# ska-sa/dc_sand

Hardware: AMD Instinct MI355X
Metric: Gcoeff/s (complex weights) 64ant x 1024beam x 32768chan per GPU (higher is better)
Workload: dtype f32

## Files before the change

dc_sand_amd/csrc/bf_capi.hip:

```cpp

#include "../../include/dcs_beamformer.h"
#ifdef DCS_PROBES
#include "../../include/dcs_probes.h"
#endif

#include <hip/hip_runtime.h>

#include <cmath>
#include <cstdio>
#include <cstdlib>
#include <cstring>
#include <new>

#include "../../include/dcs_stream_staging.h"
#include "bf_kernels.h"
#include "bf_ctx_ext.h"
#include "bf_stream_ext.h"

static_assert(sizeof(dcs_delay_vals) == 16, "delay_vals must be 4 x fp32 (BeamformerParameters.h:61-66)");

#define DCS_TRY(expr)                          \
    do {                                       \
        hipError_t _e = (expr);                \
        if (_e != hipSuccess) return (int)_e;  \
    } while (0)

namespace {

constexpr uint32_t kDtSlotFloats = 4096;
constexpr int kDtSlots = 8;

inline hipStream_t as_stream(void *s) { return reinterpret_cast<hipStream_t>(s); }

#define DCS_CHECK_DEVICE(c)                                                \
    do {                                                                   \
        int _cur = -1;                                                     \
        if (hipGetDevice(&_cur) != hipSuccess || _cur != (c)->device) return DCS_ERR_WRONG_DEVICE; \
    } while (0)

bool params_ok(const dcs_bf_params *p)
{
    if (!p) return false;
    if (p->nr_channels < 1 || p->nr_channels > (1 << 24)) return false;
    if (p->nr_stations < 1 || p->nr_beams < 1) return false;
    if ((uint64_t)p->nr_stations * (uint64_t)p->nr_beams > 0x7fffffffull) return false;
    if (!(p->sampling_period > 0.0f) || !std::isfinite(p->sampling_period)) return false;
    if (p->fft_size < 1) return false;
    if (p->nr_samples_per_channel < 1 || p->accumulations_before_new_coeffs < 1) return false;
    if (!(p->adc_sample_rate > 0.0) || !std::isfinite(p->adc_sample_rate)) return false;
    const float D = p->sampling_period * (float)p->nr_channels;
    if (!(D >= 0x1p-40f && D <= 0x1p40f)) return false;
    return true;
}

dcs_bf_consts make_consts(const dcs_bf_params *p)
{
    dcs_bf_consts k;
    volatile float D = p->sampling_period * (float)p->nr_channels;
    volatile float y = 1.0f / D;
    k.fDenominator = D;
    k.fRcpDenominator = y;
    const double scale = (double)(p->nr_channels - 1) * 3.14159274101257324219 / (double)D;
    k.fRotBoundScale = (float)(scale * 1.0001) ;
    if (!(k.fRotBoundScale >= 0.0f)) k.fRotBoundScale = INFINITY;
    k.uDiv3Exact = 0u;
    k.fLowDegLimit = 500.0f;
    k.uHalfMath = 0u;
    k.dHalfChannels = p->nr_channels / 2.0;
    k.dDenominator = (double)D;
    return k;
}

int verify_div3(dcs_bf_consts *k)
{
    uint32_t *d_cnt = nullptr;
    uint32_t h_cnt = 1;
    hipError_t e = hipMalloc((void **)&d_cnt, sizeof(uint32_t));
    if (e != hipSuccess) return (int)e;
    e = hipMemset(d_cnt, 0, sizeof(uint32_t));
    if (e == hipSuccess) e = bf_launch_verify_div3(k->fDenominator, k->fRcpDenominator, d_cnt, nullptr);
    if (e == hipSuccess) e = hipMemcpy(&h_cnt, d_cnt, sizeof(uint32_t), hipMemcpyDeviceToHost);
    (void)hipFree(d_cnt);
    if (e != hipSuccess) return (int)e;
    k->uDiv3Exact = (h_cnt == 0u) ? 1u : 0u;
    return DCS_OK;
}

}

constexpr int kSideStreams = 4;
struct dcs_bf_context {
    bf_ctx_ext_head ext;
    dcs_bf_params p;
    dcs_bf_consts k;
    uint32_t n_pairs;
    int device;
    uint32_t div3_verified;
    bool tuning_now;
    dcs_delay_vals *d_table[2];
    int cur;
    bool table_set;
    float *d_dt;
    float *h_dt;
    hipEvent_t dt_ev[kDtSlots];
    hipStream_t side[kSideStreams];
    hipEvent_t fork_ev, join_ev[kSideStreams];
    bool dt_used[kDtSlots];
    int dt_next;
    uint32_t pairs_pad;
    uint32_t terms_steps;
    float *d_terms;
    uint32_t *d_flags;
    uint32_t flag_epoch;
    float *d_wnorm;
    float *d_wscale;
    float *d_tt_terms;
    uint32_t *d_tt_flags;
    dcs_bf_tuning tune;
    struct tuned_geom {
        bool valid;
        int32_t tpb, cpb, wpc;
    } tuned[3][2];
#ifdef DCS_PROBES
    dcs_probe_knobs probe;
#endif
};
#ifdef DCS_PROBES
#define DCS_PROBE_KNOB(c, f) ((c)->probe.f)
#else
#define DCS_PROBE_KNOB(c, f) 0
#endif

constexpr int kTableRing = 4;
struct dcs_bf_stream {
    bf_stream_ext_head ext;
    dcs_bf_context *ctx;
    hipStream_t stream;
    hipGraph_t graph;
    hipGraphExec_t exec;
    hipGraphNode_t node;
    bf_kernel_launch launch;
    bool has_terms;
    hipGraphNode_t terms_node;
    bf_terms_args terms_args;
    const void *terms_func;
    dim3 terms_grid, terms_block;
    dcs_delay_vals *h_table[kTableRing];
    hipEvent_t table_copied[kTableRing];
    bool table_pending[kTableRing];
    int table_next;
    hipGraph_t ggraph;
    hipGraphExec_t gexec;
    hipGraphNode_t gnode_gather, gnode_terms, gnode_gen;
    bf_gather_launch gather;
    dcs_delay_vals *d_spare;
    hipStream_t stage_stream;
    hipEvent_t staged_ev;
    hipEvent_t released_ev;
    bool released_recorded;
    bool staged;
};

extern "C" {

const char *dcs_error_string(int status)
{
    switch (status) {
    case DCS_OK: return "dcs: success";
    case DCS_ERR_INVALID_ARGUMENT: return "dcs error: invalid argument";
    case DCS_ERR_UNSUPPORTED: return "dcs error: this kernel does not support the requested mode";
    case DCS_ERR_NOT_READY: return "dcs error: not ready (no delay table set)";
    case DCS_ERR_OUT_OF_RANGE: return "dcs error: out of range";
    case DCS_ERR_NO_DEVICE: return "dcs error: no HIP device";
    case DCS_ERR_WRONG_DEVICE: return "dcs error: the context belongs to another device than the current one (dcs_device_set)";
    default: break;
    }
    if (status > 0) return hipGetErrorString((hipError_t)status);
    return "dcs error: unknown status";
}

int dcs_abi_version(void) { return DCS_BF_ABI_VERSION; }

int dcs_bf_default_params(dcs_bf_params *p)
{
    if (!p) return DCS_ERR_INVALID_ARGUMENT;
    p->nr_channels = 64;
    p->nr_stations = 64;
    p->nr_beams = 16;
    p->nr_samples_per_channel = 256;
    p->sampling_period = 1e-7f;
    p->fft_size = 8192;
    p->adc_sample_rate = 1712e6;
    p->accumulations_before_new_coeffs = 256;
    p->reserved = 0;
    return DCS_OK;
}

int dcs_bf_output_bytes(const dcs_bf_params *p, int bitwidth, uint32_t nt, size_t *bytes)
{
    if (!params_ok(p) || !bytes) return DCS_ERR_INVALID_ARGUMENT;
    if (bitwidth != DCS_BF_B16 && bitwidth != DCS_BF_B32) return DCS_ERR_INVALID_ARGUMENT;
    const size_t elem = bitwidth == DCS_BF_B16 ? sizeof(uint16_t) : sizeof(float);
    *bytes = (size_t)nt * (size_t)p->nr_channels * (size_t)p->nr_stations * (size_t)p->nr_beams * 2u * elem;
    return DCS_OK;
}

int dcs_bf_delta_times(const dcs_bf_params *p, uint64_t t0, uint32_t nt, float *dt_out)
{
    if (!params_ok(p) || (!dt_out && nt)) return DCS_ERR_INVALID_ARGUMENT;
    for (uint32_t i = 0; i < nt; i++) {
        const uint64_t t = t0 + i;
        volatile float a = (float)t;
        volatile float b = a * p->sampling_period;
        volatile float c = b * 1e9f;
        volatile float d = c * (float)p->fft_size;
        if (!(d < 9.2e18f)) return DCS_ERR_OUT_OF_RANGE;
        const long step_ns = (long)d;
        volatile float num = (float)step_ns;
        volatile float q = num / 1e9f;
        volatile float dt = 0.0f + q;
        dt_out[i] = dt;
    }
    return DCS_OK;
}

int dcs_bf_ts_diff(const struct timespec *first, const struct timespec *last, float *dt_out)
{
    if (!first || !last || !dt_out) return DCS_ERR_INVALID_ARGUMENT;
    volatile float fl = (float)last->tv_sec, ff = (float)first->tv_sec;
    volatile float secs = fl - ff;
    const long nanosec_difference = last->tv_nsec - first->tv_nsec;
    volatile float num = (float)nanosec_difference;
    volatile float q = num / 1e9f;
    volatile float dt = secs + q;
    *dt_out = dt;
    return DCS_OK;
}

int dcs_bf_simulate_input(const dcs_bf_params *p, dcs_delay_vals *out)
{
    if (!params_ok(p) || !out) return DCS_ERR_INVALID_ARGUMENT;
    const size_t n = (size_t)p->nr_stations * (size_t)p->nr_beams;
    for (size_t i = 0; i < n; i++) {
        volatile float ratio = (float)i / (float)n;
        volatile float ramp = ratio * p->sampling_period;
        out[i].fDelay_s = (float)((double)ramp / 3.0);
        out[i].fDelayRate_sps = (float)2e-6;
        volatile float inv = 1.0f - ratio;
        volatile float ramp2 = inv * p->sampling_period;
        out[i].fPhase_rad = (float)((double)ramp2 / 3.0);
        out[i].fPhaseRate_radps = (float)3e-6;
    }
    return DCS_OK;
}

int dcs_device_count(int *count)
{
    if (!count) return DCS_ERR_INVALID_ARGUMENT;
    *count = 0;
    hipError_t e = hipGetDeviceCount(count);
    if (e == hipErrorNoDevice) { *count = 0; return DCS_OK; }
    return (int)e;
}
int dcs_device_set(int device) { return (int)hipSetDevice(device); }
int dcs_device_synchronize(void) { return (int)hipDeviceSynchronize(); }
int dcs_device_name(int device, char *buf, size_t buflen)
{
    if (!buf || buflen == 0) return DCS_ERR_INVALID_ARGUMENT;
    hipDeviceProp_t prop;
    DCS_TRY(hipGetDeviceProperties(&prop, device));
    std::snprintf(buf, buflen, "%s (%s, %d CUs)", prop.name, prop.gcnArchName, prop.multiProcessorCount);
    return DCS_OK;
}
int dcs_malloc(void **dptr, size_t bytes)
{
    if (!dptr) return DCS_ERR_INVALID_ARGUMENT;
    return (int)hipMalloc(dptr, bytes);
}
int dcs_free(void *dptr) { return (int)hipFree(dptr); }
int dcs_host_alloc(void **hptr, size_t bytes)
{
    if (!hptr) return DCS_ERR_INVALID_ARGUMENT;
    return (int)hipHostMalloc(hptr, bytes, hipHostMallocDefault);
}
int dcs_host_free(void *hptr) { return (int)hipHostFree(hptr); }
int dcs_memcpy_htod(void *dptr, const void *hptr, size_t bytes, void *stream)
{
    return (int)hipMemcpyAsync(dptr, hptr, bytes, hipMemcpyHostToDevice, as_stream(stream));
}
int dcs_memcpy_dtoh(void *hptr, const void *dptr, size_t bytes, void *stream)
{
    return (int)hipMemcpyAsync(hptr, dptr, bytes, hipMemcpyDeviceToHost, as_stream(stream));
}
int dcs_memcpy_dtod(void *dst, const void *src, size_t bytes, void *stream)
{
    return (int)hipMemcpyAsync(dst, src, bytes, hipMemcpyDeviceToDevice, as_stream(stream));
}
int dcs_memcpy2d_dtoh(void *hptr, size_t dst_pitch, const void *dptr, size_t src_pitch, size_t row_bytes,
                      size_t nrows, void *stream)
{
    return (int)hipMemcpy2DAsync(hptr, dst_pitch, dptr, src_pitch, row_bytes, nrows, hipMemcpyDeviceToHost,
                                 as_stream(stream));
}
int dcs_memset(void *dptr, int value, size_t bytes, void *stream)
{
    return (int)hipMemsetAsync(dptr, value, bytes, as_stream(stream));
}
int dcs_stream_create(void **stream)
{
    if (!stream) return DCS_ERR_INVALID_ARGUMENT;
    hipStream_t s;
    DCS_TRY(hipStreamCreateWithFlags(&s, hipStreamNonBlocking));
    *stream = s;
    return DCS_OK;
}
int dcs_stream_destroy(void *stream) { return (int)hipStreamDestroy(as_stream(stream)); }
int dcs_stream_synchronize(void *stream) { return (int)hipStreamSynchronize(as_stream(stream)); }

int dcs_event_create(void **event)
{
    if (!event) return DCS_ERR_INVALID_ARGUMENT;
    hipEvent_t e;
    DCS_TRY(hipEventCreate(&e));
    *event = e;
    return DCS_OK;
}
int dcs_event_destroy(void *event) { return (int)hipEventDestroy(reinterpret_cast<hipEvent_t>(event)); }
int dcs_event_record(void *event, void *stream)
{
    return (int)hipEventRecord(reinterpret_cast<hipEvent_t>(event), as_stream(stream));
}
int dcs_event_synchronize(void *event) { return (int)hipEventSynchronize(reinterpret_cast<hipEvent_t>(event)); }
int dcs_event_elapsed_ms(void *start, void *stop, float *ms)
{
    if (!ms) return DCS_ERR_INVALID_ARGUMENT;
    return (int)hipEventElapsedTime(ms, reinterpret_cast<hipEvent_t>(start), reinterpret_cast<hipEvent_t>(stop));
}

namespace {
int prepare_tiled(dcs_bf_context *c, bool out16, const float *dt_dev, float dt0, uint32_t nt, uint32_t c0, uint32_t nc, void *d_out,
                  bf_kernel_launch *l, const float *dt_host, bool terms_table);
int generate_and_beamform_weighted_impl(dcs_bf_context *c, const float *dt, uint64_t t0, uint32_t nt, const int8_t *d_antenna,
                                        size_t antenna_bytes, const float *d_weights, float *d_beams, size_t beams_bytes,
                                        void *stream);
int beamform_accumulated_weighted_impl(dcs_bf_context *c, const float *dt_coeff, uint64_t t_coeff, uint32_t nt,
                                       const int8_t *d_antenna, size_t antenna_bytes, const float *d_weights, float *d_beams,
                                       size_t beams_bytes, void *stream);
const bf_ctx_ext_ops kWeightsOps = {BF_CTX_EXT_VERSION, generate_and_beamform_weighted_impl, beamform_accumulated_weighted_impl};
}

int dcs_bf_create(const dcs_bf_params *p, dcs_bf_context **out)
{
    if (!out) return DCS_ERR_INVALID_ARGUMENT;
    *out = nullptr;
    if (!params_ok(p)) return DCS_ERR_INVALID_ARGUMENT;
    int ndev = 0;
    if (hipGetDeviceCount(&ndev) != hipSuccess || ndev < 1) return DCS_ERR_NO_DEVICE;
    dcs_bf_context *c = new (std::nothrow) dcs_bf_context();
    if (!c) return (int)hipErrorOutOfMemory;
    std::memset(c, 0, sizeof(*c));
    c->ext.ops = &kWeightsOps;
    c->p = *p;
    c->k = make_consts(p);
    c->n_pairs = (uint32_t)p->nr_stations * (uint32_t)p->nr_beams;
    c->pairs_pad = (c->n_pairs + 255u) & ~255u;
    {
        const uint64_t per_step = (uint64_t)c->pairs_pad * 8u;
        uint64_t steps = (64ull << 20) / per_step;
        if (steps < 1) steps = 1;
        if (steps > kDtSlotFloats) steps = kDtSlotFloats;
        c->terms_steps = (uint32_t)steps;
    }
    c->tune.nontemporal = -1;
    c->tune.xcd_remap = -1;
    c->tune.rows_same_tile = -1;
    int st = DCS_OK;
    do {
        if ((st = (int)hipGetDevice(&c->device)) != 0) break;
        if ((st = (int)bf_warm_module()) != 0) break;
        if ((st = (int)bf_warm_module_mfma()) != 0) break;
        const size_t tb = (size_t)c->n_pairs * sizeof(dcs_delay_vals);
        if ((st = (int)hipMalloc((void **)&c->d_table[0], tb)) != 0) break;
        if ((st = (int)hipMalloc((void **)&c->d_table[1], tb)) != 0) break;
        const size_t db = (size_t)kDtSlots * kDtSlotFloats * sizeof(float);
        if ((st = (int)hipMalloc((void **)&c->d_dt, db)) != 0) break;
        if ((st = (int)hipMalloc((void **)&c->d_tt_terms, (size_t)kTermsInline * c->pairs_pad * 8u)) != 0) break;
        if ((st = (int)hipMalloc((void **)&c->d_tt_flags, (size_t)kTermsInline * (c->pairs_pad / 64u) * 4u)) != 0) break;
        if ((st = (int)hipHostMalloc((void **)&c->h_dt, db, hipHostMallocDefault)) != 0) break;
        for (int i = 0; i < kDtSlots && st == 0; i++) st = (int)hipEventCreateWithFlags(&c->dt_ev[i], hipEventDisableTiming);
        if (st != 0) break;
        for (int i = 0; i < kSideStreams && st == 0; i++) {
            st = (int)hipStreamCreateWithFlags(&c->side[i], hipStreamNonBlocking);
            if (st == 0) st = (int)hipEventCreateWithFlags(&c->join_ev[i], hipEventDisableTiming);
        }
        if (st == 0) st = (int)hipEventCreateWithFlags(&c->fork_ev, hipEventDisableTiming);
        if (st != 0) break;
        c->h_dt[0] = 0.0f;
        if ((st = (int)hipMemcpy(c->d_dt, c->h_dt, sizeof(float), hipMemcpyHostToDevice)) != 0) break;
        if ((st = verify_div3(&c->k)) != 0) break;
        c->div3_verified = c->k.uDiv3Exact;
        for (int w = 0; w < 2; w++) {
            bf_kernel_launch l;
            const uint32_t nt_all = (uint32_t)(c->p.nr_samples_per_channel < (int)kDtInline ? c->p.nr_samples_per_channel : (int)kDtInline);
            float dts[kDtInline] = {0.0f};
            if (prepare_tiled(c, w == 1, nullptr, 0.0f, nt_all > 0 ? nt_all : 1u, 0, (uint32_t)c->p.nr_channels, nullptr, &l, dts, false) == DCS_OK && l.func) {
                hipFuncAttributes attr;
                (void)hipFuncGetAttributes(&attr, l.func);
            }
        }
    } while (0);
    if (st != 0) {
        dcs_bf_destroy(c);
        return st;
    }
    *out = c;
    return DCS_OK;
}

int dcs_bf_destroy(dcs_bf_context *c)
{
    if (!c) return DCS_OK;
    (void)hipFree(c->d_table[0]);
    (void)hipFree(c->d_table[1]);
    (void)hipFree(c->d_dt);
    (void)hipFree(c->d_terms);
    (void)hipFree(c->d_flags);
    (void)hipFree(c->d_wnorm);
    (void)hipFree(c->d_wscale);
    (void)hipFree(c->d_tt_terms);
    (void)hipFree(c->d_tt_flags);
    if (c->h_dt) (void)hipHostFree(c->h_dt);
    for (int i = 0; i < kDtSlots; i++)
        if (c->dt_ev[i]) (void)hipEventDestroy(c->dt_ev[i]);
    for (int i = 0; i < kSideStreams; i++) {
        if (c->join_ev[i]) (void)hipEventDestroy(c->join_ev[i]);
        if (c->side[i]) (void)hipStreamDestroy(c->side[i]);
    }
    if (c->fork_ev) (void)hipEventDestroy(c->fork_ev);
    delete c;
    return DCS_OK;
}

int dcs_bf_upload_delays(dcs_bf_context *c, const dcs_delay_vals *table, void *stream)
{
    if (!c || !table) return DCS_ERR_INVALID_ARGUMENT;
    DCS_CHECK_DEVICE(c);
    const int nxt = c->table_set ? (c->cur ^ 1) : c->cur;
    DCS_TRY(hipMemcpyAsync(c->d_table[nxt], table, (size_t)c->n_pairs * sizeof(dcs_delay_vals),
                           hipMemcpyHostToDevice, as_stream(stream)));
    c->cur = nxt;
    c->table_set = true;
    return DCS_OK;
}

int dcs_bf_set_delays_from_global(dcs_bf_context *c, const void *d_global, uint32_t nb_total,
                                  uint32_t beam_offset, void *stream)
{
    if (!c || !d_global) return DCS_ERR_INVALID_ARGUMENT;
    DCS_CHECK_DEVICE(c);
    if ((uint64_t)beam_offset + (uint64_t)c->p.nr_beams > nb_total) return DCS_ERR_OUT_OF_RANGE;
    if ((reinterpret_cast<uintptr_t>(d_global) & 15u) != 0) return DCS_ERR_INVALID_ARGUMENT;
    const int nxt = c->table_set ? (c->cur ^ 1) : c->cur;
// ... 691 lines not shown
    a.k = c->k;
    a.fp32_chain = (c->tune.math_mode & 8) ? 1u : 0u;
#ifdef DCS_PROBES
    auto knob = [](int32_t v, const char *env) { const char *e = std::getenv(env); return (uint32_t)(v ? v : (e ? std::atoi(e) : 0)); };
    a.max_rounds = knob(c->probe.bacc_rounds, "DCS_BACC_ROUNDS");
    a.probe = knob(c->probe.bacc_probe, "DCS_BACC_PROBE");
    a.unstaged = knob(c->probe.bacc_unstaged, "DCS_BACC_UNSTAGED");
    a.plain_stores = knob(c->probe.bacc_plain, "DCS_BACC_PLAIN");
    a.no_share = knob(c->probe.bacc_no_share, "DCS_BACC_NOSHARE");
    a.wg_per_cu = knob(c->probe.bacc_wg_per_cu, "DCS_BACC_WPC");
    a.order = knob(c->probe.bacc_order, "DCS_BACC_ORDER");
    a.nbt_force = knob(c->probe.bacc_nbt, "DCS_BACC_NBT");
    a.nw_force = knob(c->probe.bacc_waves, "DCS_BACC_WAVES");
#endif
    return (int)(d_weights ? bf_launch_beamform_acc_weighted(a, wa, s) : bf_launch_beamform_acc(a, s));
}

int generate_and_beamform_weighted_impl(dcs_bf_context *c, const float *dt, uint64_t t0, uint32_t nt, const int8_t *d_antenna,
                                        size_t antenna_bytes, const float *d_weights, float *d_beams, size_t beams_bytes,
                                        void *stream)
{
    if (!c || !weights_ok(d_weights)) return DCS_ERR_INVALID_ARGUMENT;
    if (!dt && t0 % 16u) return DCS_ERR_INVALID_ARGUMENT;
    return beamform_impl(c, dt_source{dt, dt ? 0 : t0}, nt, d_antenna, antenna_bytes, d_beams, beams_bytes, stream, d_weights);
}

int beamform_accumulated_weighted_impl(dcs_bf_context *c, const float *dt_coeff, uint64_t t_coeff, uint32_t nt,
                                       const int8_t *d_antenna, size_t antenna_bytes, const float *d_weights, float *d_beams,
                                       size_t beams_bytes, void *stream)
{
    if (!c || !weights_ok(d_weights)) return DCS_ERR_INVALID_ARGUMENT;
    return beamform_acc_impl(c, dt_source{dt_coeff, dt_coeff ? 0 : t_coeff}, nt, d_antenna, antenna_bytes, d_beams, beams_bytes,
                             stream, d_weights);
}
}

int dcs_bf_beamform_accumulated(dcs_bf_context *c, uint64_t t_coeff, uint32_t nt, const int8_t *d_antenna, size_t antenna_bytes,
                                float *d_beams, size_t beams_bytes, void *stream)
{
    return beamform_acc_impl(c, dt_source{nullptr, t_coeff}, nt, d_antenna, antenna_bytes, d_beams, beams_bytes, stream);
}

int dcs_bf_beamform_accumulated_dt(dcs_bf_context *c, float dt_coeff, uint32_t nt, const int8_t *d_antenna, size_t antenna_bytes,
                                   float *d_beams, size_t beams_bytes, void *stream)
{
    return beamform_acc_impl(c, dt_source{&dt_coeff, 0}, nt, d_antenna, antenna_bytes, d_beams, beams_bytes, stream);
}

int dcs_bf_autotune(dcs_bf_context *c, int bitwidth, void *d_out, size_t out_bytes, void *stream,
                    dcs_bf_tuning *chosen)
{
    if (!c || !d_out) return DCS_ERR_INVALID_ARGUMENT;
    DCS_CHECK_DEVICE(c);
    if (bitwidth != DCS_BF_B16 && bitwidth != DCS_BF_B32) return DCS_ERR_INVALID_ARGUMENT;
    if (!c->table_set) return DCS_ERR_NOT_READY;
    const bool out16 = bitwidth == DCS_BF_B16;
    const size_t row = (size_t)c->n_pairs * (out16 ? 4u : 8u);
    uint64_t nc64 = out_bytes / row;
    if (nc64 > (uint64_t)c->p.nr_channels) nc64 = (uint64_t)c->p.nr_channels;
    if (nc64 == 0) return DCS_ERR_INVALID_ARGUMENT;
    const uint32_t nc = (uint32_t)nc64;
    uint64_t nt64 = out_bytes / (row * nc);
    if (nt64 > kDtInline) nt64 = kDtInline;
    const uint32_t nt_tune = nc == (uint32_t)c->p.nr_channels && nt64 > 1 ? (uint32_t)nt64 : 1u;
    hipStream_t s = as_stream(stream);
    {
        const int cap = refuse_if_capturing(s);
        if (cap != DCS_OK) return cap;
    }
    dcs_bf_context::tuned_geom &slot =
        c->tuned[tuned_slot(c, out16)][want_terms_table(c, out16, shape_default_geometry(c, out16, nc, nt_tune), nc, nt_tune) ? 1 : 0];

    auto report = [&]() {
        if (!chosen) return;
        *chosen = c->tune;
        chosen->tiles_per_block = slot.tpb;
        chosen->chan_per_block = slot.cpb;
        chosen->wg_per_cu = slot.wpc;
        chosen->nontemporal = 1;
    };
    if (slot.valid) {
        report();
        return DCS_OK;
    }

    struct cand { int tpb, cpb, wpc; double best_ms; };
    static const int k32[][3] = {{1, 6, -1}, {1, 7, -1}, {1, 8, -1}, {1, 9, -1}, {1, 10, -1}, {1, 11, -1}, {1, 12, -1}, {1, 13, -1},
                                 {1, 14, -1}, {1, 16, -1}, {1, 7, 7}, {1, 8, 7}, {1, 9, 7}, {1, 10, 7}, {1, 11, 7}, {1, 12, 7},
                                 {1, 13, 7}, {1, 7, 6}, {1, 8, 6}, {1, 9, 6}, {1, 10, 6}, {1, 11, 6}, {1, 12, 6}, {1, 13, 6},
                                 {1, 14, 6}, {1, 8, 5}, {1, 9, 5}, {1, 10, 5}, {1, 11, 5}, {1, 12, 5}, {1, 14, 5}, {1, 16, 5}, {2, 6, -1}, {2, 8, -1}};
    static const int k16[][3] = {{1, 16, -1}, {1, 24, -1}, {1, 32, -1}, {1, 48, -1}, {1, 64, -1}, {1, 96, -1}, {1, 128, -1},
                                 {1, 192, -1}, {1, 256, -1}, {1, 24, 6}, {1, 32, 6}, {1, 48, 6}, {1, 64, 6}, {1, 32, 7},
                                 {1, 64, 7}, {1, 128, 7}, {2, 32, -1}, {2, 64, -1},
                                 {1, 16, 6}, {1, 16, 7}, {1, 20, 5}, {1, 20, 6}, {1, 24, 4}, {1, 24, 5}, {1, 28, 4}, {1, 28, 5}, {1, 32, 4},
                                 {1, 32, 5}, {1, 40, 4}};
    const int(*tab)[3] = out16 ? k16 : k32;
    int ncand = out16 ? (int)(sizeof(k16) / sizeof(k16[0])) : (int)(sizeof(k32) / sizeof(k32[0]));
    cand cands[40];
    static_assert(sizeof(k32) / sizeof(k32[0]) < 40 && sizeof(k16) / sizeof(k16[0]) < 40, "cands[] too small");
    for (int i = 0; i < ncand; i++) cands[i] = {tab[i][0], tab[i][1], tab[i][2], 1e30};
    const bf_geom dflt = shape_default_geometry(c, out16, nc, nt_tune);
    int i_default = -1;
    for (int i = 0; i < ncand; i++)
        if (cands[i].tpb == dflt.tpb && cands[i].cpb == (int)dflt.cpb && (cands[i].wpc > 0 ? cands[i].wpc : 0) == dflt.wpc) i_default = i;
    if (i_default < 0) {
        i_default = ncand;
        cands[ncand++] = {dflt.tpb, (int)dflt.cpb, dflt.wpc > 0 ? dflt.wpc : -1, 1e30};
    }

    if (tiled_blocks(c->n_pairs, out16, dflt.tpb, dflt.cpb, nc, nt_tune) <= 256u * 8u) {
        slot.valid = true;
        slot.tpb = dflt.tpb;
        slot.cpb = (int32_t)dflt.cpb;
        slot.wpc = dflt.wpc > 0 ? dflt.wpc : -1;
        report();
        return DCS_OK;
    }
    const dcs_bf_tuning saved = c->tune;
    c->tuning_now = true;
    auto use = [&](const cand &k) {
        c->tune.form = saved.form == 2 ? 0 : saved.form;
        c->tune.tiles_per_block = k.tpb;
        c->tune.chan_per_block = k.cpb;
        c->tune.wg_per_cu = k.wpc;
        c->tune.nontemporal = 1;
    };
    hipEvent_t e0 = nullptr, e1 = nullptr;
    int st = (int)hipEventCreate(&e0);
    if (st == 0) st = (int)hipEventCreate(&e1);
    auto time_launches = [&](int n, float *ms) -> int {
        int r = (int)hipEventRecord(e0, s);
        for (int k = 0; k < n && r == 0; k++) r = dcs_bf_generate_slab(c, bitwidth, 1, nt_tune, 0, nc, d_out, out_bytes, stream);
        if (r == 0) r = (int)hipEventRecord(e1, s);
        if (r == 0) r = (int)hipEventSynchronize(e1);
        if (r == 0) r = (int)hipEventElapsedTime(ms, e0, e1);
        return r;
    };
    float cal_ms = 0.0f;
    for (int i = 0; i < 10 && st == 0; i++) st = dcs_bf_generate_slab(c, bitwidth, 1, nt_tune, 0, nc, d_out, out_bytes, stream);
    if (st == 0) st = time_launches(4, &cal_ms);
    const double one = cal_ms > 0.0f ? cal_ms / 4.0 : 1.0;
    const int n_settle = (int)std::fmin(400.0, std::fmax(8.0, std::ceil(20.0 / one)));
    const int n_timed = (int)std::fmin(200.0, std::fmax(4.0, std::ceil(3.0 / one)));
    for (int rnd = 0; rnd < 2 && st == 0; rnd++) {
        double best_so_far = 1e30;
        for (int i = 0; i < ncand; i++) best_so_far = std::fmin(best_so_far, cands[i].best_ms);
        for (int i = 0; i < ncand && st == 0; i++) {
            if (rnd == 1 && i != i_default && cands[i].best_ms > 1.04 * best_so_far) continue;
            use(cands[i]);
            for (int k = 0; k < n_settle && st == 0; k++) st = dcs_bf_generate_slab(c, bitwidth, 1, nt_tune, 0, nc, d_out, out_bytes, stream);
            float ms = 0.0f;
            if (st == 0) st = time_launches(n_timed, &ms);
            if (st == 0 && ms / n_timed < cands[i].best_ms) cands[i].best_ms = ms / n_timed;
        }
    }
    int order[40];
    for (int i = 0; i < ncand; i++) order[i] = i;
    for (int i = 0; i < ncand; i++)
        for (int j = i + 1; j < ncand; j++)
            if (cands[order[j]].best_ms < cands[order[i]].best_ms) { const int t = order[i]; order[i] = order[j]; order[j] = t; }
    int finalists[5];
    int nfinal = 0;
    for (int i = 0; i < ncand && nfinal < 4; i++)
        if (order[i] != i_default) finalists[nfinal++] = order[i];
    finalists[nfinal++] = i_default;
    double final_ms[5] = {0.0, 0.0, 0.0, 0.0, 0.0};
    const int n_final = (int)std::fmin(800.0, std::fmax(8.0, std::ceil(12.0 / one)));
    for (int rnd = 0; rnd < 3 && st == 0; rnd++) {
        for (int f = 0; f < nfinal && st == 0; f++) {
            use(cands[finalists[f]]);
            for (int i = 0; i < n_settle && st == 0; i++) st = dcs_bf_generate_slab(c, bitwidth, 1, nt_tune, 0, nc, d_out, out_bytes, stream);
            float ms = 0.0f;
            if (st == 0) st = time_launches(n_final, &ms);
            final_ms[f] += ms / n_final;
        }
    }
    if (e0) (void)hipEventDestroy(e0);
    if (e1) (void)hipEventDestroy(e1);
    int best = i_default;
    double best_ms = final_ms[nfinal - 1] / 1.007;
    for (int f = 0; f + 1 < nfinal && st == 0; f++)
        if (final_ms[f] < best_ms) { best_ms = final_ms[f]; best = finalists[f]; }
    if (st == 0) {
        use(cands[best]);
        for (int k = 0; k < n_settle && st == 0; k++) st = dcs_bf_generate_slab(c, bitwidth, 1, nt_tune, 0, nc, d_out, out_bytes, stream);
    }
    c->tune = saved;
    c->tuning_now = false;
    if (st != 0) return st;
    slot.valid = true;
    slot.tpb = cands[best].tpb;
    slot.cpb = cands[best].cpb;
    slot.wpc = cands[best].wpc;
    report();
    return DCS_OK;
}

int dcs_bf_gpu_utilisation(const dcs_bf_params *p, float kernel_ms, float out[2])
{
    if (!params_ok(p) || !out) return DCS_ERR_INVALID_ARGUMENT;
    const float fRateOfFFTs_Hz = ((float)p->adc_sample_rate) / ((float)p->fft_size);
    const float fTransferTimePerPacket_s = 1 / fRateOfFFTs_Hz;
    float single = (kernel_ms / 1000.0) / (p->nr_samples_per_channel * fTransferTimePerPacket_s);
    float multiple = single / ((float)p->accumulations_before_new_coeffs);
    single *= 4;
    multiple *= 4;
    out[0] = single;
    out[1] = multiple;
    return DCS_OK;
}

namespace {

void kernel_node_params(const bf_kernel_launch &l, void **params, hipKernelNodeParams *np)
{
    std::memset(np, 0, sizeof(*np));
    np->func = const_cast<void *>(l.func);
    np->gridDim = l.grid;
    np->blockDim = l.block;
    np->sharedMemBytes = l.shared;
    np->kernelParams = params;
    np->extra = nullptr;
}

void terms_node_params(const dcs_bf_stream *s, void **params, hipKernelNodeParams *tp)
{
    std::memset(tp, 0, sizeof(*tp));
    tp->func = const_cast<void *>(s->terms_func);
    tp->gridDim = s->terms_grid;
    tp->blockDim = s->terms_block;
    tp->kernelParams = params;
}

void gather_node_params(dcs_bf_stream *s, void **params, hipKernelNodeParams *gp)
{
    bf_gather_launch &g = s->gather;
    params[0] = &g.local;
    params[1] = &g.global;
    params[2] = &g.n_ant;
    params[3] = &g.nb_local;
    params[4] = &g.nb_total;
    params[5] = &g.beam_offset;
    std::memset(gp, 0, sizeof(*gp));
    gp->func = const_cast<void *>(g.func);
    gp->gridDim = g.grid;
    gp->blockDim = g.block;
    gp->kernelParams = params;
}

int build_stream_graph(dcs_bf_stream *s, bool with_gather, hipGraph_t *graph, hipGraphExec_t *exec, hipGraphNode_t *n_gather,
                       hipGraphNode_t *n_terms, hipGraphNode_t *n_gen)
{
    DCS_TRY(hipGraphCreate(graph, 0));
    hipGraphNode_t prev = nullptr;
    if (with_gather) {
        void *gparams[6];
        hipKernelNodeParams gp;
        gather_node_params(s, gparams, &gp);
        DCS_TRY(hipGraphAddKernelNode(n_gather, *graph, nullptr, 0, &gp));
        prev = *n_gather;
    }
    if (s->has_terms) {
        void *tparams[] = {&s->terms_args};
        hipKernelNodeParams tp;
        terms_node_params(s, tparams, &tp);
        DCS_TRY(hipGraphAddKernelNode(n_terms, *graph, prev ? &prev : nullptr, prev ? 1 : 0, &tp));
        prev = *n_terms;
    }
    void *params[] = {&s->launch.args};
    hipKernelNodeParams np;
    kernel_node_params(s->launch, params, &np);
    DCS_TRY(hipGraphAddKernelNode(n_gen, *graph, prev ? &prev : nullptr, prev ? 1 : 0, &np));
    DCS_TRY(hipGraphInstantiate(exec, *graph, nullptr, nullptr, 0));
    return DCS_OK;
}

int replay(dcs_bf_stream *s, float dt, const dcs_delay_vals *delays, hipGraphExec_t exec, hipGraphNode_t n_gather,
           hipGraphNode_t n_terms, hipGraphNode_t n_gen)
{
    s->launch.args.a.dt0 = dt;
    s->launch.args.a.delays = delays;
    if (n_gather) {
        void *gparams[6];
        hipKernelNodeParams gp;
        gather_node_params(s, gparams, &gp);
        DCS_TRY(hipGraphExecKernelNodeSetParams(exec, n_gather, &gp));
    }
    if (s->has_terms) {
        s->terms_args.dt0 = dt;
        s->terms_args.dt_inline[0] = dt;
        s->terms_args.delays = delays;
        void *tparams[] = {&s->terms_args};
        hipKernelNodeParams tp;
        terms_node_params(s, tparams, &tp);
        DCS_TRY(hipGraphExecKernelNodeSetParams(exec, n_terms, &tp));
    }
    void *params[] = {&s->launch.args};
    hipKernelNodeParams np;
    kernel_node_params(s->launch, params, &np);
    DCS_TRY(hipGraphExecKernelNodeSetParams(exec, n_gen, &np));
    return (int)hipGraphLaunch(exec, s->stream);
}

int ensure_staging(dcs_bf_stream *s)
{
    if (!s->d_spare) DCS_TRY(hipMalloc((void **)&s->d_spare, (size_t)s->ctx->n_pairs * sizeof(dcs_delay_vals)));
    if (!s->stage_stream) {
        int least = 0, greatest = 0;
        DCS_TRY(hipDeviceGetStreamPriorityRange(&least, &greatest));
        DCS_TRY(hipStreamCreateWithPriority(&s->stage_stream, hipStreamNonBlocking, greatest));
    }
    if (!s->staged_ev) DCS_TRY(hipEventCreateWithFlags(&s->staged_ev, hipEventDisableTiming));
    if (!s->released_ev) DCS_TRY(hipEventCreateWithFlags(&s->released_ev, hipEventDisableTiming));
    return DCS_OK;
}

int begin_staging(dcs_bf_stream *s)
{
    const int cap = refuse_if_capturing(s->stream);
    if (cap != DCS_OK) return cap;
    const int st = ensure_staging(s);
    if (st != DCS_OK) return st;
    if (s->released_recorded) DCS_TRY(hipStreamWaitEvent(s->stage_stream, s->released_ev, 0));
    return DCS_OK;
}

int consume_staged(dcs_bf_stream *s, float dt)
{
    dcs_bf_context *c = s->ctx;
    DCS_TRY(hipStreamWaitEvent(s->stream, s->staged_ev, 0));
    DCS_TRY(hipEventRecord(s->released_ev, s->stream));
    s->released_recorded = true;
    const int st = replay(s, dt, s->d_spare, s->exec, nullptr, s->terms_node, s->node);
    if (st != DCS_OK) return st;
    dcs_delay_vals *retired = c->d_table[c->cur];
    c->d_table[c->cur] = s->d_spare;
    s->d_spare = retired;
    s->staged = false;
    return DCS_OK;
}

int stage_table_impl(dcs_bf_stream *s, const dcs_delay_vals *table, int flags)
{
    if (!s || !table) return DCS_ERR_INVALID_ARGUMENT;
    if (flags != 0 && flags != DCS_BF_STAGE_CALLER_PINNED) return DCS_ERR_INVALID_ARGUMENT;
    dcs_bf_context *c = s->ctx;
    DCS_CHECK_DEVICE(c);
    const size_t tb = (size_t)c->n_pairs * sizeof(dcs_delay_vals);
    const int st = begin_staging(s);
    if (st != DCS_OK) return st;
    const void *src = table;
    int r = -1;
    if (flags == 0) {
        r = s->table_next;
        s->table_next = (r + 1) % kTableRing;
        if (s->table_pending[r]) DCS_TRY(hipEventSynchronize(s->table_copied[r]));
        std::memcpy(s->h_table[r], table, tb);
        src = s->h_table[r];
    }
    DCS_TRY(hipMemcpyAsync(s->d_spare, src, tb, hipMemcpyHostToDevice, s->stage_stream));
    if (r >= 0) {
        DCS_TRY(hipEventRecord(s->table_copied[r], s->stage_stream));
        s->table_pending[r] = true;
    }
    DCS_TRY(hipEventRecord(s->staged_ev, s->stage_stream));
    s->staged = true;
    return DCS_OK;
}

int stage_table_from_global_impl(dcs_bf_stream *s, const void *d_global, uint32_t nb_total, uint32_t beam_offset,
                                 void *ready_event)
{
    if (!s || !d_global) return DCS_ERR_INVALID_ARGUMENT;
    dcs_bf_context *c = s->ctx;
    DCS_CHECK_DEVICE(c);
    if ((uint64_t)beam_offset + (uint64_t)c->p.nr_beams > nb_total) return DCS_ERR_OUT_OF_RANGE;
    if ((reinterpret_cast<uintptr_t>(d_global) & 15u) != 0) return DCS_ERR_INVALID_ARGUMENT;
    const int st = begin_staging(s);
    if (st != DCS_OK) return st;
    if (ready_event) DCS_TRY(hipStreamWaitEvent(s->stage_stream, reinterpret_cast<hipEvent_t>(ready_event), 0));
    DCS_TRY(bf_launch_gather_beams(s->d_spare, static_cast<const dcs_delay_vals *>(d_global), (uint32_t)c->p.nr_stations,
                                   (uint32_t)c->p.nr_beams, nb_total, beam_offset, s->stage_stream));
    DCS_TRY(hipEventRecord(s->staged_ev, s->stage_stream));
    s->staged = true;
    return DCS_OK;
}

const bf_stream_ext_ops kStagingOps = {BF_STREAM_EXT_VERSION, stage_table_impl, stage_table_from_global_impl};

}

int dcs_bf_stream_begin(dcs_bf_context *c, int bitwidth, uint32_t c0, uint32_t nc, void *d_out, size_t out_bytes,
                        void *stream, dcs_bf_stream **out)
{
    if (!c || !out || !d_out) return DCS_ERR_INVALID_ARGUMENT;
    DCS_CHECK_DEVICE(c);
    *out = nullptr;
    if (bitwidth != DCS_BF_B16 && bitwidth != DCS_BF_B32) return DCS_ERR_INVALID_ARGUMENT;
    if (!c->table_set) return DCS_ERR_NOT_READY;
    if ((uint64_t)c0 + nc > (uint64_t)c->p.nr_channels || nc == 0) return DCS_ERR_OUT_OF_RANGE;
    const bool out16 = bitwidth == DCS_BF_B16;
    if (out_bytes < (size_t)nc * c->n_pairs * (out16 ? 4 : 8)) return DCS_ERR_INVALID_ARGUMENT;
    {
        const int cap = refuse_if_capturing(as_stream(stream));
        if (cap != DCS_OK) return cap;
    }

    dcs_bf_stream *s = new (std::nothrow) dcs_bf_stream();
    if (!s) return (int)hipErrorOutOfMemory;
    std::memset(static_cast<void *>(s), 0, sizeof(*s));
    s->ext.ops = &kStagingOps;
    s->ctx = c;
    s->stream = as_stream(stream);
    int st = DCS_OK;
    do {
        s->has_terms = want_terms_table(c, out16, pick_geometry(c, out16, nc, 1), nc, 1);
        if ((st = prepare_tiled(c, out16, nullptr, 0.0f, 1, c0, nc, d_out, &s->launch, nullptr, s->has_terms)) != 0) break;
        if (s->launch.func == nullptr) { st = DCS_ERR_INVALID_ARGUMENT; break; }
        if (s->has_terms) {
            fill_terms_table_args(c, out16, 0.0f, 1, c0, nc, d_out, nullptr, &s->terms_args);
            if ((st = (int)bf_prepare_terms(s->terms_args, &s->terms_func, &s->terms_grid, &s->terms_block)) != 0) break;
            if (s->terms_func == nullptr) { st = DCS_ERR_INVALID_ARGUMENT; break; }
        }
        if ((st = (int)bf_prepare_gather_beams(c->d_table[c->cur ^ 1], c->d_table[c->cur], (uint32_t)c->p.nr_stations,
                                               (uint32_t)c->p.nr_beams, (uint32_t)c->p.nr_beams, 0u, &s->gather)) != 0) break;
        if (s->gather.func == nullptr) { st = DCS_ERR_INVALID_ARGUMENT; break; }
        for (int i = 0; i < kTableRing && st == 0; i++) {
            st = (int)hipHostMalloc((void **)&s->h_table[i], (size_t)c->n_pairs * sizeof(dcs_delay_vals), hipHostMallocDefault);
            if (st == 0) st = (int)hipEventCreateWithFlags(&s->table_copied[i], hipEventDisableTiming);
        }
        if (st != 0) break;
        if ((st = build_stream_graph(s, false, &s->graph, &s->exec, nullptr, &s->terms_node, &s->node)) != 0) break;
        if ((st = build_stream_graph(s, true, &s->ggraph, &s->gexec, &s->gnode_gather, &s->gnode_terms, &s->gnode_gen)) != 0) break;
    } while (0);
    if (st != 0) {
        dcs_bf_stream_end(s);
        return st;
    }
    *out = s;
    return DCS_OK;
}

int dcs_bf_stream_tick_dt(dcs_bf_stream *s, float dt, const dcs_delay_vals *new_table)
{
    if (!s) return DCS_ERR_INVALID_ARGUMENT;
    dcs_bf_context *c = s->ctx;
    DCS_CHECK_DEVICE(c);
    if (s->staged) return new_table ? DCS_ERR_INVALID_ARGUMENT : consume_staged(s, dt);
    if (new_table) {
        const int r = s->table_next;
        s->table_next = (r + 1) % kTableRing;
        if (s->table_pending[r]) DCS_TRY(hipEventSynchronize(s->table_copied[r]));
        std::memcpy(s->h_table[r], new_table, (size_t)c->n_pairs * sizeof(dcs_delay_vals));
        const int nxt = c->cur ^ 1;
        DCS_TRY(hipMemcpyAsync(c->d_table[nxt], s->h_table[r], (size_t)c->n_pairs * sizeof(dcs_delay_vals),
                               hipMemcpyHostToDevice, s->stream));
        DCS_TRY(hipEventRecord(s->table_copied[r], s->stream));
        s->table_pending[r] = true;
        c->cur = nxt;
    }
    return replay(s, dt, c->d_table[c->cur], s->exec, nullptr, s->terms_node, s->node);
}

int dcs_bf_stream_tick(dcs_bf_stream *s, uint64_t t, const dcs_delay_vals *new_table)
{
    if (!s) return DCS_ERR_INVALID_ARGUMENT;
    float dt;
    const int st = dcs_bf_delta_times(&s->ctx->p, t, 1, &dt);
    if (st != DCS_OK) return st;
    return dcs_bf_stream_tick_dt(s, dt, new_table);
}

int dcs_bf_stream_tick_at(dcs_bf_stream *s, const struct timespec *cur, const struct timespec *ref,
                          const dcs_delay_vals *new_table)
{
    if (!s) return DCS_ERR_INVALID_ARGUMENT;
    float dt;
    const int st = dcs_bf_ts_diff(ref, cur, &dt);
    if (st != DCS_OK) return st;
    return dcs_bf_stream_tick_dt(s, dt, new_table);
}

int dcs_bf_stream_tick_dt_from_global(dcs_bf_stream *s, float dt, const void *d_global, uint32_t nb_total, uint32_t beam_offset)
{
    if (!s || !d_global) return DCS_ERR_INVALID_ARGUMENT;
    dcs_bf_context *c = s->ctx;
    DCS_CHECK_DEVICE(c);
    if ((uint64_t)beam_offset + (uint64_t)c->p.nr_beams > nb_total) return DCS_ERR_OUT_OF_RANGE;
    if ((reinterpret_cast<uintptr_t>(d_global) & 15u) != 0) return DCS_ERR_INVALID_ARGUMENT;
    if (s->staged) return DCS_ERR_INVALID_ARGUMENT;
    const int nxt = c->cur ^ 1;
    s->gather.local = c->d_table[nxt];
    s->gather.global = static_cast<const dcs_delay_vals *>(d_global);
    s->gather.nb_total = nb_total;
    s->gather.beam_offset = beam_offset;
    c->cur = nxt;
    return replay(s, dt, c->d_table[c->cur], s->gexec, s->gnode_gather, s->gnode_terms, s->gnode_gen);
}

int dcs_bf_stream_tick_from_global(dcs_bf_stream *s, uint64_t t, const void *d_global, uint32_t nb_total, uint32_t beam_offset)
{
    if (!s) return DCS_ERR_INVALID_ARGUMENT;
    float dt;
    const int st = dcs_bf_delta_times(&s->ctx->p, t, 1, &dt);
    if (st != DCS_OK) return st;
    return dcs_bf_stream_tick_dt_from_global(s, dt, d_global, nb_total, beam_offset);
}

int dcs_bf_stream_tick_at_from_global(dcs_bf_stream *s, const struct timespec *cur, const struct timespec *ref,
                                      const void *d_global, uint32_t nb_total, uint32_t beam_offset)
{
    if (!s) return DCS_ERR_INVALID_ARGUMENT;
    float dt;
    const int st = dcs_bf_ts_diff(ref, cur, &dt);
    if (st != DCS_OK) return st;
    return dcs_bf_stream_tick_dt_from_global(s, dt, d_global, nb_total, beam_offset);
}

int dcs_bf_stream_end(dcs_bf_stream *s)
{
    if (!s) return DCS_OK;
    (void)hipStreamSynchronize(s->stream);
    if (s->stage_stream) {
        (void)hipStreamSynchronize(s->stage_stream);
        (void)hipStreamDestroy(s->stage_stream);
    }
    if (s->staged_ev) (void)hipEventDestroy(s->staged_ev);
    if (s->released_ev) (void)hipEventDestroy(s->released_ev);
    if (s->d_spare) (void)hipFree(s->d_spare);
    if (s->exec) (void)hipGraphExecDestroy(s->exec);
    if (s->graph) (void)hipGraphDestroy(s->graph);
    if (s->gexec) (void)hipGraphExecDestroy(s->gexec);
    if (s->ggraph) (void)hipGraphDestroy(s->ggraph);
    for (int i = 0; i < kTableRing; i++) {
        if (s->table_copied[i]) (void)hipEventDestroy(s->table_copied[i]);
        if (s->h_table[i]) (void)hipHostFree(s->h_table[i]);
    }
    delete s;
    return DCS_OK;
}

#ifdef DCS_PROBES
int dcs_probe_set_knobs(dcs_bf_context *c, const dcs_probe_knobs *k)
{
    if (!c) return DCS_ERR_INVALID_ARGUMENT;
    if (!k) {
        std::memset(&c->probe, 0, sizeof(c->probe));
        return DCS_OK;
    }
    if (k->pace < 0 || k->pace > 4096 || k->fail_at_step < 0) return DCS_ERR_INVALID_ARGUMENT;
    c->probe = *k;
    return DCS_OK;
}
#endif

}
```

Measured before the change: 914.9.

## Use a growable pool of spare device tables for staged delay uploads

Replaces the single spare device delay table with a pool of up to 16 buffers, each with its own release event, so staging a new table no longer has to wait for the previous generation kernel to release the spare. Non-capturing tick calls with a host table are routed through the staging path on the high-priority side stream instead of copying on the main stream. The aim is to let table uploads overlap the beamformer kernel rather than serialize with it. The cost is extra device memory and more event bookkeeping. It also fixes the ordering of the cur update on replay failure in the gather path.

```diff
diff --git a/dc_sand_amd/csrc/bf_capi.hip b/dc_sand_amd/csrc/bf_capi.hip
--- a/dc_sand_amd/csrc/bf_capi.hip
+++ b/dc_sand_amd/csrc/bf_capi.hip
@@ -132,6 +132,7 @@
 #endif
 
 constexpr int kTableRing = 4;
+constexpr int kSparePool = 16;
 struct dcs_bf_stream {
     bf_stream_ext_head ext;
     dcs_bf_context *ctx;
@@ -153,11 +154,15 @@
     hipGraphExec_t gexec;
     hipGraphNode_t gnode_gather, gnode_terms, gnode_gen;
     bf_gather_launch gather;
-    dcs_delay_vals *d_spare;
+    struct spare_table {
+        dcs_delay_vals *buf;
+        hipEvent_t free_ev;
+        bool recorded;
+    } spare[kSparePool];
+    int n_spare;
+    int spare_cur;
     hipStream_t stage_stream;
     hipEvent_t staged_ev;
-    hipEvent_t released_ev;
-    bool released_recorded;
     bool staged;
 };
 
@@ -1455,16 +1460,34 @@
     return (int)hipGraphLaunch(exec, s->stream);
 }
 
+int add_spare(dcs_bf_stream *s, int at)
+{
+    dcs_bf_stream::spare_table t = {nullptr, nullptr, false};
+    DCS_TRY(hipMalloc((void **)&t.buf, (size_t)s->ctx->n_pairs * sizeof(dcs_delay_vals)));
+    const hipError_t e = hipEventCreateWithFlags(&t.free_ev, hipEventDisableTiming);
+    if (e != hipSuccess) {
+        (void)hipFree(t.buf);
+        return (int)e;
+    }
+    for (int i = s->n_spare; i > at; i--) s->spare[i] = s->spare[i - 1];
+    s->spare[at] = t;
+    s->n_spare++;
+    return DCS_OK;
+}
+
 int ensure_staging(dcs_bf_stream *s)
 {
-    if (!s->d_spare) DCS_TRY(hipMalloc((void **)&s->d_spare, (size_t)s->ctx->n_pairs * sizeof(dcs_delay_vals)));
+    if (s->n_spare == 0) {
+        const int st = add_spare(s, 0);
+        if (st != DCS_OK) return st;
+        s->spare_cur = 0;
+    }
     if (!s->stage_stream) {
         int least = 0, greatest = 0;
         DCS_TRY(hipDeviceGetStreamPriorityRange(&least, &greatest));
         DCS_TRY(hipStreamCreateWithPriority(&s->stage_stream, hipStreamNonBlocking, greatest));
     }
     if (!s->staged_ev) DCS_TRY(hipEventCreateWithFlags(&s->staged_ev, hipEventDisableTiming));
-    if (!s->released_ev) DCS_TRY(hipEventCreateWithFlags(&s->released_ev, hipEventDisableTiming));
     return DCS_OK;
 }
 
@@ -1474,21 +1497,36 @@
     if (cap != DCS_OK) return cap;
     const int st = ensure_staging(s);
     if (st != DCS_OK) return st;
-    if (s->released_recorded) DCS_TRY(hipStreamWaitEvent(s->stage_stream, s->released_ev, 0));
+    if (s->staged) return DCS_OK;
+    int next = (s->spare_cur + 1) % s->n_spare;
+    if (s->spare[next].recorded) {
+        const hipError_t q = hipEventQuery(s->spare[next].free_ev);
+        if (q == hipSuccess) {
+            s->spare[next].recorded = false;
+        } else if (q != hipErrorNotReady) {
+            return (int)q;
+        } else if (s->n_spare < kSparePool && add_spare(s, s->spare_cur + 1) == DCS_OK) {
+            next = s->spare_cur + 1;
+        } else {
+            DCS_TRY(hipStreamWaitEvent(s->stage_stream, s->spare[next].free_ev, 0));
+        }
+    }
+    s->spare_cur = next;
     return DCS_OK;
 }
 
 int consume_staged(dcs_bf_stream *s, float dt)
 {
     dcs_bf_context *c = s->ctx;
+    dcs_bf_stream::spare_table &t = s->spare[s->spare_cur];
     DCS_TRY(hipStreamWaitEvent(s->stream, s->staged_ev, 0));
-    DCS_TRY(hipEventRecord(s->released_ev, s->stream));
-    s->released_recorded = true;
-    const int st = replay(s, dt, s->d_spare, s->exec, nullptr, s->terms_node, s->node);
+    DCS_TRY(hipEventRecord(t.free_ev, s->stream));
+    const int st = replay(s, dt, t.buf, s->exec, nullptr, s->terms_node, s->node);
     if (st != DCS_OK) return st;
     dcs_delay_vals *retired = c->d_table[c->cur];
-    c->d_table[c->cur] = s->d_spare;
-    s->d_spare = retired;
+    c->d_table[c->cur] = t.buf;
+    t.buf = retired;
+    t.recorded = true;
     s->staged = false;
     return DCS_OK;
 }
@@ -1511,7 +1549,7 @@
         std::memcpy(s->h_table[r], table, tb);
         src = s->h_table[r];
     }
-    DCS_TRY(hipMemcpyAsync(s->d_spare, src, tb, hipMemcpyHostToDevice, s->stage_stream));
+    DCS_TRY(hipMemcpyAsync(s->spare[s->spare_cur].buf, src, tb, hipMemcpyHostToDevice, s->stage_stream));
     if (r >= 0) {
         DCS_TRY(hipEventRecord(s->table_copied[r], s->stage_stream));
         s->table_pending[r] = true;
@@ -1532,7 +1570,7 @@
     const int st = begin_staging(s);
     if (st != DCS_OK) return st;
     if (ready_event) DCS_TRY(hipStreamWaitEvent(s->stage_stream, reinterpret_cast<hipEvent_t>(ready_event), 0));
-    DCS_TRY(bf_launch_gather_beams(s->d_spare, static_cast<const dcs_delay_vals *>(d_global), (uint32_t)c->p.nr_stations,
+    DCS_TRY(bf_launch_gather_beams(s->spare[s->spare_cur].buf, static_cast<const dcs_delay_vals *>(d_global), (uint32_t)c->p.nr_stations,
                                    (uint32_t)c->p.nr_beams, nb_total, beam_offset, s->stage_stream));
     DCS_TRY(hipEventRecord(s->staged_ev, s->stage_stream));
     s->staged = true;
@@ -1601,6 +1639,15 @@
     DCS_CHECK_DEVICE(c);
     if (s->staged) return new_table ? DCS_ERR_INVALID_ARGUMENT : consume_staged(s, dt);
     if (new_table) {
+        hipStreamCaptureStatus cs = hipStreamCaptureStatusNone;
+        DCS_TRY(hipStreamIsCapturing(s->stream, &cs));
+        if (cs == hipStreamCaptureStatusNone) {
+            int st = stage_table_impl(s, new_table, 0);
+            if (st != DCS_OK) return st;
+            st = consume_staged(s, dt);
+            if (st != DCS_OK) s->staged = false;
+            return st;
+        }
         const int r = s->table_next;
         s->table_next = (r + 1) % kTableRing;
         if (s->table_pending[r]) DCS_TRY(hipEventSynchronize(s->table_copied[r]));
@@ -1647,8 +1694,9 @@
     s->gather.global = static_cast<const dcs_delay_vals *>(d_global);
     s->gather.nb_total = nb_total;
     s->gather.beam_offset = beam_offset;
-    c->cur = nxt;
-    return replay(s, dt, c->d_table[c->cur], s->gexec, s->gnode_gather, s->gnode_terms, s->gnode_gen);
+    const int st = replay(s, dt, c->d_table[nxt], s->gexec, s->gnode_gather, s->gnode_terms, s->gnode_gen);
+    if (st == DCS_OK) c->cur = nxt;
+    return st;
 }
 
 int dcs_bf_stream_tick_from_global(dcs_bf_stream *s, uint64_t t, const void *d_global, uint32_t nb_total, uint32_t beam_offset)
@@ -1679,8 +1727,10 @@
         (void)hipStreamDestroy(s->stage_stream);
     }
     if (s->staged_ev) (void)hipEventDestroy(s->staged_ev);
-    if (s->released_ev) (void)hipEventDestroy(s->released_ev);
-    if (s->d_spare) (void)hipFree(s->d_spare);
+    for (int i = 0; i < s->n_spare; i++) {
+        (void)hipEventDestroy(s->spare[i].free_ev);
+        (void)hipFree(s->spare[i].buf);
+    }
     if (s->exec) (void)hipGraphExecDestroy(s->exec);
     if (s->graph) (void)hipGraphDestroy(s->graph);
     if (s->gexec) (void)hipGraphExecDestroy(s->gexec);
```

Result: no change. 913.6 (-0.1%).
